# taindp98/Endoscopy-Image-Classification

Measured on AMD Instinct MI355X. Metric: unlabeled images/sec/node (FixMatch ViT-S, 224², μ=7), higher is better.
Workload: dtype bf16; 1 GPU; F1: FixMatch ViT-S/16 step, global B=64 labeled + mu*B=448 unlabeled weak/strong pairs (64 + 448 per GPU, strong scaling), 224^2, C=23, tau=0.95, lambda_u=1, Adam 1e-3, EMA 0.999; global_batch=960, seq_len=197, parallelism=dp1, hipgraph=False

## Files before the change

### endoscopy-image-classification_amd/csrc/gemm.hip

```cpp
#include <algorithm>
#include <mutex>
#include <type_traits>

#include <hip/hip_ext.h>

#include "common.h"

namespace es_gemm {

constexpr int BM = 128, BN = 128, BK = 64;

enum Epi {
  EPI_BF16 = 0,
  EPI_GELU = 1,
  EPI_F32_RESID = 2,
  EPI_DGELU = 3,
  EPI_F32 = 4,
  EPI_PATCH = 5,
  EPI_GELU_ACT = 6,
  EPI_GELU_D = 7,
  EPI_MULAUX = 8,
};

struct NTArgs {
// ... 1405 lines not shown
        }
        if constexpr (s == 0)
          if (q == RPS / 2 - 1) load_resid(std::integral_constant<int, 3>{});
        const LnRow384 o = ln_row384(v, (q & 1) == 0, l.eps, gam_lds, bet_lds, lane);
        const int m = m0 + tile_row(s, q);
        const bool ok = m < p.M;
#pragma unroll
        for (int j = 0; j < 3; ++j) {
          const int c = (j * 64 + lane) * 2;
          __builtin_amdgcn_raw_buffer_store_b64(__builtin_bit_cast(u32x2, v[j]), rx,
                                                ok ? (unsigned)(m * p.ldc + c) * 4u : ES_OOB, 0, 0);
          __builtin_amdgcn_raw_buffer_store_b32(o.h[j], rh, ok ? (unsigned)(m * l.ldh + c) * 2u : ES_OOB, 0, 0);
        }
        const bool one = ok && lane == 0;
        __builtin_amdgcn_raw_buffer_store_b32(__builtin_bit_cast(unsigned, o.mean), rm,
                                              one ? (unsigned)m * 4u : ES_OOB, 0, 0);
        __builtin_amdgcn_raw_buffer_store_b32(__builtin_bit_cast(unsigned, o.rstd), rs,
                                              one ? (unsigned)m * 4u : ES_OOB, 0, 0);
      }
    };
    slab(std::integral_constant<int, 0>{});
    asm volatile("s_waitcnt lgkmcnt(0)" ::: "memory");
    __builtin_amdgcn_s_barrier();
    slab(std::integral_constant<int, 1>{});
    if (tid == 0) qslot[0] = claimed;
    asm volatile("s_waitcnt lgkmcnt(0)" ::: "memory");
    __builtin_amdgcn_s_barrier();
    cur = __builtin_amdgcn_readfirstlane(qslot[0]);
  }
  TILE_CTR_RELEASE(ctr, tid)
}
#undef TILE_CTR_RELEASE

#define NT_LAUNCH(E, BKT_, NST_, TBM_, ...)                                             \
  {                                                                                        \
    const size_t lds = std::max((size_t)NST_ * (TBM_ + BN) * BKT_ * 2, (size_t)4 * EPI_WAVE_BYTES); \
    allow_lds(gemm_nt_kernel<E, BKT_, NST_, TBM_, ##__VA_ARGS__>, lds);                   \
    hipLaunchKernelGGL(HIP_KERNEL_NAME(gemm_nt_kernel<E, BKT_, NST_, TBM_, ##__VA_ARGS__>), dim3(grid), dim3(256), lds, stream, a); \
    return ES_OK;                                                                          \
  }
#define NT_EPIS(BKT_, NST_, TBM_, ...)                                            \
  switch (epi) {                                                                  \
    case EPI_BF16: NT_LAUNCH(EPI_BF16, BKT_, NST_, TBM_, ##__VA_ARGS__)           \
    case EPI_GELU: NT_LAUNCH(EPI_GELU, BKT_, NST_, TBM_, ##__VA_ARGS__)           \
    case EPI_F32_RESID: NT_LAUNCH(EPI_F32_RESID, BKT_, NST_, TBM_, ##__VA_ARGS__) \
    case EPI_DGELU: NT_LAUNCH(EPI_DGELU, BKT_, NST_, TBM_, ##__VA_ARGS__)         \
    case EPI_F32: NT_LAUNCH(EPI_F32, BKT_, NST_, TBM_, ##__VA_ARGS__)             \
    case EPI_PATCH: NT_LAUNCH(EPI_PATCH, BKT_, NST_, TBM_, ##__VA_ARGS__)         \
    case EPI_GELU_ACT: NT_LAUNCH(EPI_GELU_ACT, BKT_, NST_, TBM_, ##__VA_ARGS__)   \
    case EPI_GELU_D: NT_LAUNCH(EPI_GELU_D, BKT_, NST_, TBM_, ##__VA_ARGS__)       \
    case EPI_MULAUX: NT_LAUNCH(EPI_MULAUX, BKT_, NST_, TBM_, ##__VA_ARGS__)       \
    default: return ES_BAD_ARG;                                                   \
  }
int launch_nt(int cfg, int epi, int grid, hipStream_t stream, const NTArgs& a) {
  if (cfg == 11 && epi == EPI_F32_RESID) NT_LAUNCH(EPI_F32_RESID, 64, 2, 64, 0)
  switch (cfg) {
    case 0: NT_EPIS(64, 2, 128)
    case 5: NT_EPIS(32, 2, 128)
    case 11: NT_EPIS(64, 2, 64)
    default: NT_EPIS(32, 3, 128)
  }
}
#undef NT_EPIS
#undef NT_LAUNCH

#define BIG_LAUNCH(E, WM_, MF_, NF_, NST_, BKT_, OCC_, ...)                                        \
// ... 39 lines not shown
  if (n < CTR_SLOTS) {
    tab[n] = s;
    return n++;
  }
  return (int)(((uintptr_t)s >> 6) % CTR_SLOTS);
}
static int persistent_grid(int tiles) {
  static const int cus = [] {
    int dev = 0, n = 0;
    (void)hipGetDevice(&dev);
    return (hipDeviceGetAttribute(&n, hipDeviceAttributeMultiprocessorCount, dev) != hipSuccess || n <= 0) ? 256 : n;
  }();
  return std::max(1, std::min(cus, tiles));
}

int launch_resid_ln(hipStream_t stream, const NTArgs& a, const RLArgs& l) {
  const int grid = persistent_grid((a.M + rlg::R - 1) / rlg::R);
  allow_lds(gemm_resid_ln_kernel, (size_t)rlg::LDS);
  hipLaunchKernelGGL(gemm_resid_ln_kernel, dim3(grid), dim3(512), rlg::LDS, stream, a, l, tile_ctr_slot(stream));
  return hipGetLastError() == hipSuccess ? ES_OK : ES_HIP_ERROR;
}

int launch_nt_ln(int ring, hipStream_t stream, const NTArgs& a, const RLArgs& l) {
  const int grid = persistent_grid((a.M + nlg::TBM - 1) / nlg::TBM);
  const int slot = tile_ctr_slot(stream);
  constexpr size_t lds3 = nlg::lds<3, 32>(), lds2 = nlg::lds<2, 64>();
  if (ring == 1) {
    allow_lds(gemm_nt_ln_kernel<3, 32>, lds3);
    hipLaunchKernelGGL(HIP_KERNEL_NAME(gemm_nt_ln_kernel<3, 32>), dim3(grid), dim3(512), lds3, stream, a, l, slot);
  } else {
    allow_lds(gemm_nt_ln_kernel<2, 64>, lds2);
    hipLaunchKernelGGL(HIP_KERNEL_NAME(gemm_nt_ln_kernel<2, 64>), dim3(grid), dim3(512), lds2, stream, a, l, slot);
  }
  return hipGetLastError() == hipSuccess ? ES_OK : ES_HIP_ERROR;
}

}
using namespace es_gemm;

static int g_gemm_variant = -1;
static int g_tn_variant = -1;
static int g_small_tile = 1;

extern "C" {

int es_gemm_tn_ex(const void* A1, int ld1, const void* A2, int ld2, int M, int N1, int N2, int splits,
                  float* workspace, float* out, int accumulate, float* bias_out, int variant, hipStream_t stream);

int es_gemm_nt(int epi, const void* A, int lda, const void* B, int ldb, const float* bias, void* C,
               int ldc, void* C2, const void* aux, int ldaux, int M, int N, int K, int np,
               hipStream_t stream) {
  if (M <= 0 || N <= 0 || K <= 0 || (N % BN) || (K % BK) || (lda % 8) || (ldb % 8) || (ldc % 4))
    return ES_BAD_SHAPE;
  if (!A || !B || !C) return ES_BAD_ARG;
  if (((epi == EPI_GELU || epi == EPI_GELU_D) && !C2) ||
      ((epi == EPI_F32_RESID || epi == EPI_DGELU || epi == EPI_MULAUX || epi == EPI_PATCH) && !aux))
    return ES_BAD_ARG;
  if (epi == EPI_PATCH && np <= 0) return ES_BAD_ARG;
  if ((epi == EPI_F32_RESID || epi == EPI_PATCH) && ((ldaux % 4) || ldaux < N)) return ES_BAD_SHAPE;
  if ((epi == EPI_DGELU || epi == EPI_MULAUX) && ((ldaux % 8) || ldaux < N)) return ES_BAD_SHAPE;
  NTArgs a{(const bf16*)A, (const bf16*)B, bias, C, C2, aux, M, N, K, lda, ldb, ldc, ldaux, np};
  int variant = g_gemm_variant;
  if (variant < 0) {
    const bool gelu = epi == EPI_GELU || epi == EPI_GELU_ACT || epi == EPI_GELU_D;
    const bool plain = epi == EPI_BF16 || epi == EPI_F32 || epi == EPI_F32_RESID || epi == EPI_MULAUX;
    if (g_small_tile && N <= 384 && ((K <= 384 && epi == EPI_F32_RESID) || (M < 32768 && (plain || epi == EPI_GELU_ACT))))
// ... 56 lines not shown
      (size_t)M * (size_t)std::max(ldc, ldaux) * 4 >= (1u << 31))
    return ES_BAD_SHAPE;
  if (!A || !B || !C || !aux || !gamma || !beta || !h || !mean || !rstd) return ES_BAD_ARG;
  if ((((uintptr_t)A | (uintptr_t)aux | (uintptr_t)B | (uintptr_t)gamma | (uintptr_t)beta) & 15) ||
      (bias && ((uintptr_t)bias & 15)) || ((uintptr_t)C & 7) || ((uintptr_t)h & 3))
    return ES_BAD_ARG;
  NTArgs a{(const bf16*)A, (const bf16*)B, bias, C, nullptr, aux, M, N, K, lda, ldb, ldc, ldaux, 0};
  RLArgs l{gamma, beta, (bf16*)h, mean, rstd, ldh, eps};
  return launch_resid_ln(stream, a, l);
}

static int g_nt_ln_ring = 0;
int es_gemm_nt_ln(const void* A, int lda, const void* B, int ldb, const float* bias, float* C, int ldc,
                  const float* aux, int ldaux, const float* gamma, const float* beta, void* h, int ldh, float* mean,
                  float* rstd, int M, int N, int K, float eps, hipStream_t stream) {
  if (M <= 0 || N != nlg::D || K <= 0 || (K % 64) || (lda % 8) || (ldb % 8) || (ldc % 2) || (ldaux % 2) || (ldh % 2) ||
      lda < K || ldb < K || ldc < N || ldaux < N || ldh < N ||
      (size_t)M * (size_t)std::max(std::max(ldc, ldaux), ldh) * 4 >= (1u << 31))
    return ES_BAD_SHAPE;
  if (!A || !B || !C || !aux || !gamma || !beta || !h || !mean || !rstd) return ES_BAD_ARG;
  if ((((uintptr_t)A | (uintptr_t)B | (uintptr_t)gamma | (uintptr_t)beta) & 15) || (bias && ((uintptr_t)bias & 15)) ||
      (((uintptr_t)C | (uintptr_t)aux) & 7) || (((uintptr_t)h | (uintptr_t)mean | (uintptr_t)rstd) & 3))
    return ES_BAD_ARG;
  NTArgs a{(const bf16*)A, (const bf16*)B, bias, C, nullptr, aux, M, N, K, lda, ldb, ldc, ldaux, 0};
  RLArgs l{gamma, beta, (bf16*)h, mean, rstd, ldh, eps};
  return launch_nt_ln(g_nt_ln_ring, stream, a, l);
}
int endossl_nt_ln_ring(int v) {
  const int old = g_nt_ln_ring;
  g_nt_ln_ring = v == 1 ? 1 : 0;
  return old;
}

static bool gemm_variant_ok(int v) {
  return v == -1 || v == 0 || v == 1 || v == 2 || v == 5 || v == 6 || v == 10 || v == 11;
}
int es_set_gemm_variant(int v) {
  if (!gemm_variant_ok(v)) return ES_BAD_ARG;
  const int old = g_gemm_variant;
  g_gemm_variant = v;
  return old;
}

int es_set_gemm_small_tile(int v) {
  const int old = g_small_tile;
  g_small_tile = v;
  return old;
}

int es_set_tn_variant(int v) {
  if (v != -1 && v != 0 && v != 7) return ES_BAD_ARG;
  const int old = g_tn_variant;
  g_tn_variant = v;
  return old;
}

constexpr int TN_MIN_SPLIT_TOKENS = 512;
static bool tn_big_ok(int N1, int N2, int ld1, int ld2) {
  return N1 % TB1 == 0 && N2 % TB2 == 0 && ld1 % 8 == 0 && ld2 % 8 == 0;
}
static int tn_pick(int M, int N1, int N2, int ld1, int ld2, int v) {
  if (!(N1 % BM == 0 && N2 % BN == 0)) return 7;
  if (v == 7) return tn_big_ok(N1, N2, ld1, ld2) ? 7 : 0;
  if (v >= 0) return 0;
  return (tn_big_ok(N1, N2, ld1, ld2) && M >= 65536) ? 7 : 0;
}
// ... 259 lines not shown
```

### endoscopy-image-classification_amd/endossl/_lib.py

```python
import ctypes
import os

import torch

_HERE = os.path.dirname(os.path.abspath(__file__))
LIB_PATH = os.environ.get("ENDOSSL_LIB", os.path.join(_HERE, "lib", "libendossl_hip.so"))

V, I, L, F, Z = ctypes.c_void_p, ctypes.c_int, ctypes.c_long, ctypes.c_float, ctypes.c_size_t
U64 = ctypes.c_ulonglong

SIGNATURES = {
    "es_abi_version": (I, []),
    "es_gemm_nt": (I, [I, V, I, V, I, V, V, I, V, V, I, I, I, I, I, V]),
    "es_gemm_nt_resid_ln": (I, [V, I, V, I, V, V, I, V, I, V, V, V, I, V, V, I, I, I, F, V]),
    "es_gemm_nt_ln": (I, [V, I, V, I, V, V, I, V, I, V, V, V, I, V, V, I, I, I, F, V]),
    "es_set_gemm_variant": (I, [I]),
    "es_set_gemm_small_tile": (I, [I]),
    "es_gemm_tn_workspace": (Z, [I, I, I]),
    "es_gemm_tn": (I, [V, I, V, I, I, I, I, I, V, V, I, V, V]),
    "es_gemm_tn_ex": (I, [V, I, V, I, I, I, I, I, V, V, I, V, I, V]),
    "es_set_tn_variant": (I, [I]),
    "es_set_attn_variant": (I, [I]),
    "es_set_attn_bwd_variant": (I, [I]),
    "es_set_attn_bwd_grid": (I, [I]),
    "es_set_ln_fwd_grid": (I, [I]),
    "es_set_attn_bwd_long": (I, [I]),
    "es_splitk_reduce": (I, [V, V, I, I, I, V]),
    "es_tn_problem_size": (Z, []),
    "es_gemm_tn_grouped_prepare": (I, [V, I]),
    "es_gemm_tn_grouped": (I, [V, I, I, V]),
    "es_set_stem_kernels": (I, [I]),
    "es_gemm_tn_big_grouped_table_bytes": (Z, [I]),
    "es_gemm_tn_big_grouped_workspace": (Z, [V, I, I]),
    "es_gemm_tn_big_grouped_prepare": (I, [V, I, I, V, Z, V, V]),
    "es_gemm_tn_big_grouped": (I, [V, I, V, V]),
    "es_gemm_tn_big_grouped_timed": (I, [V, I, V, V, V, V]),
    "es_event_create": (I, [V]),
    "es_event_elapsed": (I, [V, V, V]),
    "es_event_destroy": (I, [V]),
    "es_colsum": (I, [V, I, I, I, V, I, V, I, V]),
    "es_attn_fwd": (I, [V, I, V, I, V, I, I, I, F, V]),
    "es_attn_bwd": (I, [V, I, V, I, V, V, V, I, V, I, I, I, I, F, V]),
    "es_attn_cls_fwd": (I, [V, I, V, I, V, I, I, I, F, V]),
    "es_attn_cls_bwd": (I, [V, I, V, I, V, V, I, V, I, I, I, I, F, V]),
    "es_reduce_partials": (I, [V, V, I, I, I, V]),
    "es_layernorm_fwd": (I, [V, I, V, V, V, I, V, V, I, I, F, V]),
    "es_layernorm_bwd": (I, [V, I, V, I, V, V, V, V, I, V, I, V, I, V, V, V, I, I, I, I, V]),
    "es_layernorm_bwd_b16": (I, [V, I, V, I, V, V, V, V, I, V, I, V, I, V, V, V, I, I, I, I, V]),
# ... 250 lines not shown
```

### endoscopy-image-classification_amd/endossl/block.py

```python
import contextlib
import ctypes

import torch

from . import _lib
from ._lib import ptr, stream

EPI_BF16, EPI_GELU, EPI_F32_RESID, EPI_DGELU, EPI_F32, EPI_PATCH, EPI_GELU_ACT, EPI_GELU_D, EPI_MULAUX = range(9)
ATTN_SCALE = 64 ** -0.5


def gemm_nt(call, epi, a, w, bias, c, M, N, K, c2=None, aux=None, ldc=None, ldaux=None, npatch=0, s=None):
    call("es_gemm_nt", epi, ptr(a), a.stride(0), ptr(w), w.stride(0), ptr(bias), ptr(c), ldc or c.stride(0), ptr(c2),
         ptr(aux), 0 if aux is None else ldaux or aux.stride(0), M, N, K, npatch, stream() if s is None else s)


def gemm_nt_resid_ln(call, a, w, bias, xmid, xin, gamma, beta, h, mean, rstd, M, N, K, eps, s=None):
    call("es_gemm_nt_resid_ln", ptr(a), a.stride(0), ptr(w), w.stride(0), ptr(bias), ptr(xmid), xmid.stride(0),
         ptr(xin), xin.stride(0), ptr(gamma), ptr(beta), ptr(h), h.stride(0), ptr(mean), ptr(rstd), M, N, K, eps,
         stream() if s is None else s)


def gemm_nt_ln(call, a, w, bias, xout, xmid, gamma, beta, h, mean, rstd, M, N, K, eps, s=None):
    call("es_gemm_nt_ln", ptr(a), a.stride(0), ptr(w), w.stride(0), ptr(bias), ptr(xout), xout.stride(0), ptr(xmid),
         xmid.stride(0), ptr(gamma), ptr(beta), ptr(h), h.stride(0), ptr(mean), ptr(rstd), M, N, K, eps,
         stream() if s is None else s)


def layernorm_fwd(call, x, gamma, beta, y, mean, rstd, M, D, eps, s=None):
    call("es_layernorm_fwd", ptr(x), x.stride(0), ptr(gamma), ptr(beta), ptr(y), y.stride(0), ptr(mean), ptr(rstd), M,
         D, eps, stream() if s is None else s)


def layernorm_bwd(call, dy, x, mean, rstd, gamma, dres, dx, dxb, dgamma, dbeta, ws, blocks, M, D, accumulate,
                  lddx=None, s=None):
    call("es_layernorm_bwd_b16" if dy.dtype == torch.bfloat16 else "es_layernorm_bwd", ptr(dy), dy.stride(0), ptr(x),
         x.stride(0), ptr(mean), ptr(rstd), ptr(gamma), ptr(dres), dres.stride(0), ptr(dx), lddx or dx.stride(0),
         ptr(dxb), 0 if dxb is None else dxb.stride(0), ptr(dgamma), ptr(dbeta), ptr(ws), blocks, M, D, accumulate,
         stream() if s is None else s)


def attn_fwd(call, qkv, o, lse, n, T, H, s=None, cls=False):
    call("es_attn_cls_fwd" if cls else "es_attn_fwd", ptr(qkv), qkv.stride(0), ptr(o), o.stride(0), ptr(lse), n, T, H,
         ATTN_SCALE, stream() if s is None else s)


def attn_bwd(call, qkv, o, lse, delta, do, dqkv, n, T, H, s=None):
    call("es_attn_bwd", ptr(qkv), qkv.stride(0), ptr(o), o.stride(0), ptr(lse), ptr(delta), ptr(do), do.stride(0),
         ptr(dqkv), dqkv.stride(0), n, T, H, ATTN_SCALE, stream() if s is None else s)


def attn_cls_bwd(call, qkv, o, lse, do, dqkv, n, T, H, s=None):
    call("es_attn_cls_bwd", ptr(qkv), qkv.stride(0), ptr(o), o.stride(0), ptr(lse), ptr(do), do.stride(0), ptr(dqkv),
         dqkv.stride(0), n, T, H, ATTN_SCALE, stream() if s is None else s)


def cast_f32_bf16(call, src, dst, numel, s=None):
    call("es_cast_f32_bf16", ptr(src), ptr(dst), numel, stream() if s is None else s)

# ... 24 lines not shown
        w, bias = self.wb[b + "attn.qkv.weight"], p(b + "attn.qkv.bias")
        if cls is not None and split_q:
            gemm_nt(call, EPI_BF16, R.h1, w[D:], bias[D:], R.qkv[:, D:], M, 2 * D, D, s=s)
            cls.h1[:R.n].copy_(R.h1[:M].view(R.n, R.T, D)[:, 0])
            gemm_nt(call, EPI_BF16, cls.h1, w[:D], bias[:D], R.qkv, R.n, D, D, ldc=R.T * 3 * D, s=s)
        else:
            gemm_nt(call, EPI_BF16, R.h1, w, bias, R.qkv, M, 3 * D, D, s=s)
        Ro = R if cls is None else cls
        attn_fwd(call, R.qkv, Ro.o, Ro.lse, R.n, R.T, self.heads, s, cls is not None)

    def mlp_fwd(self, b, R, train, fused=False, label=None, next_ln=None):
        call, p, wb, s, M = self.call, self.p, self.wb, stream(), R.rows
        D, Hd = R.h2.shape[1], R.act.shape[1]
        if fused:
            gemm_nt_resid_ln(call, R.o, wb[b + "attn.proj.weight"], p(b + "attn.proj.bias"), R.xmid, R.x,
                             p(b + "norm2.weight"), p(b + "norm2.bias"), R.h2, R.mean2, R.rstd2, M, D, D, self.eps, s)
        else:
            gemm_nt(call, EPI_F32_RESID, R.o, wb[b + "attn.proj.weight"], p(b + "attn.proj.bias"), R.xmid, M, D, D,
                    aux=R.x, ldaux=R.ldx, s=s)
            layernorm_fwd(call, R.xmid, p(b + "norm2.weight"), p(b + "norm2.bias"), R.h2, R.mean2, R.rstd2, M, D,
                          self.eps, s)
        epi, c, c2 = (EPI_GELU_D if self.gelu_d else EPI_GELU, R.pre, R.act) if train else (EPI_GELU_ACT, R.act, None)
        fc1 = lambda: gemm_nt(call, epi, R.h2, wb[b + "mlp.fc1.weight"], p(b + "mlp.fc1.bias"), c, M, Hd, D,
                              c2=c2, s=s)
        self.bracket(label, 2.0 * M * Hd * D, fc1)
        if next_ln is not None:
            gamma, beta, h1, mean1, rstd1 = next_ln
            gemm_nt_ln(call, R.act, wb[b + "mlp.fc2.weight"], p(b + "mlp.fc2.bias"), R.out, R.xmid, gamma, beta, h1,
                       mean1, rstd1, M, D, Hd, self.eps, s)
            return
        gemm_nt(call, EPI_F32_RESID, R.act, wb[b + "mlp.fc2.weight"], p(b + "mlp.fc2.bias"), R.out, M, D, Hd,
                aux=R.xmid, s=s)

    def mlp_bwd(self, b, R, ln_bwd, wgrad=None, cap=nop, label=None):
        call, p, g, wt, s, M = self.call, self.p, self.g, self.wt, stream(), R.rows
        D, Hd = R.dxb.shape[1], R.dpre.shape[1]
        cap("b_dxb", R.dxb)
        gemm_nt(call, EPI_MULAUX if self.gelu_d else EPI_DGELU, R.dxb, wt[b + "mlp.fc2.weight"], None, R.dpre, M, Hd, D,
                aux=R.pre, s=s)
        if wgrad is not None:
            wgrad(R.dxb, D, R.act, Hd, M, g(b + "mlp.fc2.weight"), g(b + "mlp.fc2.bias"))
        gemm_nt(call, self.epi_dh, R.dpre, wt[b + "mlp.fc1.weight"], None, R.dh, M, D, Hd, s=s)
        if wgrad is not None:
            wgrad(R.dpre, Hd, R.h2, D, M, g(b + "mlp.fc1.weight"), g(b + "mlp.fc1.bias"), label=label)
        cap("b_dpre", R.dpre)
        cap("b_dh2", R.dh)
        ln_bwd(R.dh, R.xmid, R.mean2, R.rstd2, p(b + "norm2.weight"), R.dres, R.dxm, R.dxmb, g(b + "norm2.weight"),
               g(b + "norm2.bias"), M, lddx=R.lddxm)
        gemm_nt(call, EPI_BF16, R.dxmb, wt[b + "attn.proj.weight"], None, R.do, M, D, D, s=s)
        if wgrad is not None:
            wgrad(R.dxmb, D, R.o, D, M, g(b + "attn.proj.weight"), g(b + "attn.proj.bias"))
        cap("b_dxm", R.dxm, R.dxmb)
        cap("b_do", R.do)

    def attn_bwd(self, b, R, ln_bwd, wgrad=None, before_ln1=nop, cap=nop, cls=None, split_q=False):
        call, p, g, s, M, T = self.call, self.p, self.g, stream(), R.rows, R.T
        D = R.dh1.shape[1]
        if cls is None:
            attn_bwd(call, R.qkv, R.o, R.lse, R.delta, R.do, R.dqkv, R.n, T, self.heads, s)
        else:
            attn_cls_bwd(call, R.qkv, cls.o, cls.lse, cls.do, R.dqkv, R.n, T, self.heads, s)
        gemm_nt(call, self.epi_dh, R.dqkv, self.wt[b + "attn.qkv.weight"], None, R.dh1, M, D, 3 * D, s=s)
        if wgrad is not None:
            gw, gb = g(b + "attn.qkv.weight"), g(b + "attn.qkv.bias")
            if cls is not None and split_q:
                wgrad(R.dqkv[:, D:], 2 * D, R.h1, D, M, gw[D * D:], gb[D:], ld1=3 * D)
                wgrad(R.dqkv, D, R.h1, D, R.n, gw[:D * D], gb[:D], ld1=T * 3 * D, ld2=T * D)
            else:
                wgrad(R.dqkv, 3 * D, R.h1, D, M, gw, gb)
        cap("b_dqkv", R.dqkv)
        cap("b_dh1", R.dh1)
        before_ln1()
        ln_bwd(R.dh1, R.x, R.mean1, R.rstd1, p(b + "norm1.weight"), R.dxm, R.dx, R.dxb_next, g(b + "norm1.weight"),
               g(b + "norm1.bias"), M)

# ... 42 lines not shown
```

### endoscopy-image-classification_amd/endossl/vit.py

```python
import ctypes
import functools
import math
import os

import torch
import torch.nn as nn

from . import _lib, block
from ._lib import call, ptr
from .block import (EPI_BF16, EPI_DGELU, EPI_F32, EPI_F32_RESID, EPI_GELU, EPI_GELU_ACT,
                    EPI_GELU_D, EPI_MULAUX, EPI_PATCH, Rows, _TNProblem)

LN_BWD_BLOCKS = 1024
SIDE_PRIORITY = -1
SIDE_PRIORITY_MIN_M = 65536


IMAGENET_MEAN = (0.485, 0.456, 0.406)
IMAGENET_STD = (0.229, 0.224, 0.225)


def _rup(x, m):
    return (x + m - 1) // m * m

# ... 213 lines not shown
            self._launch_grouped(self.problems, 0)
        if self.defer:
            self._ln_flush(self.defer)
        if self.side is not None:
            self.main.wait_stream(self.side)


class Engine:

    TN_TARGET_BLOCKS = 768
    TN_SHARE = 0.5
    TN_SHARE_MIN_M = 16384
    TN_MAX_SPLITS = 128
    GROUP_WGRAD = "auto"
    GROUP_WGRAD_MAX_M = 16384
    GROUP_LAYERS = 6
    DEFER_LN_GRADS = True
    LN_MULTI_MAX = 32
    LAYER_WGRAD = True
    LAYER_TN_SHARE = 0.375
    _OV = os.environ.get("ENDOSSL_OVERLAP", "1")
    OVERLAP_FWD = _OV in ("1", "fwd")
    OVERLAP = _OV in ("1", "bwd")
    DH_BF16 = True
    GELU_D = True
    PRUNE_LAST = True
    PRUNE_Q = True
    RESID_LN = os.environ.get("ENDOSSL_RESID_LN", "1") == "1"
    RESID_LN_MIN_M = 40000
    FC2_LN = os.environ.get("ENDOSSL_FC2_LN", "1") == "1"
    FC2_LN_MIN_M = 50000
    FC2_LN_TRAIN = True
    FC2_LN_WEAK = True

    PARITY_NAMES = {n: n + "_f32" for n in (
        "es_gemm_nt", "es_gemm_tn", "es_attn_fwd", "es_attn_bwd", "es_attn_cls_fwd", "es_attn_cls_bwd",
        "es_layernorm_fwd", "es_layernorm_bwd", "es_patch_im2col", "es_patch_im2col_u8", "es_embed_bwd",
        "es_pack_weights")}
    PARITY_NAMES.update({"es_layernorm_bwd_b16": "es_layernorm_bwd_f32", "es_cast_f32_bf16": "es_copy_f32"})

    def __init__(self, cfg, device, precision="bf16"):
        if precision not in ("bf16", "fp32"):
            raise ValueError(f"precision must be 'bf16' (production) or 'fp32' (parity mode), got {precision!r}")
        self.cfg, self.device = cfg, device
        self.precision = precision
        self.op_dtype = torch.bfloat16 if precision == "bf16" else torch.float32
        self.layout, self.offs, self.numel = param_layout(cfg)
        self.shapes = dict(self.layout)
        self._acts = {}
        self._grads = {}
        self._ws = None
        self._ws_ln = None
        self._ws_lnp = None
        self._lnp_next = 0
        self._side = None
        self._ncu_cache = None
        self._gtab = {}
        self._grad_b = None
        self.overlap = self.OVERLAP
        self.overlap_fwd = self.OVERLAP_FWD
        self._packed_version = -1
        D, Hd = cfg.dim, cfg.hidden
        b16 = self.op_dtype
        mats = [("patch_embed.proj.weight", D, 3 * cfg.patch * cfg.patch, False)]
        for i in range(cfg.depth):
            b = f"blocks.{i}."
# ... 201 lines not shown
        if defer is not None and grid >= 64:
            ws = self.ln_part_workspace(self._lnp_next)
            self._lnp_next += 1
            block.layernorm_bwd(self._call, dy, x, mean, rstd, gamma, dres, dx, dxb, None, None, ws, LN_BWD_BLOCKS, M,
                                D, 0, lddx)
            defer.append((ws, dgamma, dbeta, grid, 0))
            return
        block.layernorm_bwd(self._call, dy, x, mean, rstd, gamma, dres, dx, dxb, dgamma, dbeta, self.ln_workspace(),
                            LN_BWD_BLOCKS, M, D, 0, lddx)

    def ln_part_workspace(self, k):
        if self._ws_lnp is None:
            self._ws_lnp = []
        while len(self._ws_lnp) <= k:
            self._ws_lnp.append(torch.empty(2 * LN_BWD_BLOCKS * self.cfg.dim, dtype=torch.float32, device=self.device))
        return self._ws_lnp[k]

    def _ln_grads_flush(self, pending):
        if not pending:
            return
        lib = _lib.load()
        esz = lib.es_ln_param_grads_entry_size()
        for c0 in range(0, len(pending), self.LN_MULTI_MAX):
            chunk = pending[c0:c0 + self.LN_MULTI_MAX]
            raw = (ctypes.c_char * (esz * len(chunk)))()
            for j, (ws, dg, db, grid, acc) in enumerate(chunk):
                ent = (ctypes.c_void_p(ptr(ws)), ctypes.c_void_p(ptr(dg)), ctypes.c_void_p(ptr(db)),
                       ctypes.c_int(grid), ctypes.c_int(self.cfg.dim), ctypes.c_int(acc), ctypes.c_int(0))
                buf = b"".join(bytes(e) for e in ent)
                ctypes.memmove(ctypes.byref(raw, j * esz), buf, len(buf))
            self._call("es_ln_param_grads_multi", ctypes.addressof(raw), len(chunk), _lib.stream())
        pending.clear()

    def backward(self, flat, grad, dlogits=None, dfts=None, zero_grad=True, grad_ready=None):
        cfg = self.cfg
        s = _lib.stream()
        top = dfts if cfg.head == "emb" else dlogits
        if top is None:
            raise ValueError("Engine.backward needs dlogits (cls head) or dfts (emb head)")
        n = int(top.shape[0])
        A = self.acts(n, True)
        D, T, M = cfg.dim, cfg.T, A.M
        gv = lambda name: self.view(grad, name)
        fv = lambda name: self.view(flat, name)
        grouped = self._grouped_wgrad(M, grad_ready)
        GS = self._grad_sets(n, grouped)
        G = GS[0]
        sched = _WgradSchedule(
            GS, M, cfg.depth, grouped, layer_wgrad=self.LAYER_WGRAD, defer_ln=self.DEFER_LN_GRADS,
            bf16=self.precision == "bf16", capture=self.capture is not None, group_layers=self.GROUP_LAYERS,
            min_m=self.TN_SHARE_MIN_M, main=torch.cuda.current_stream(self.device),
            side=self.side_stream(M) if self.overlap else None, wgrad=self._wgrad, wgrad_layer=self._wgrad_layer,
            launch_grouped=self._launch_grouped, ln_flush=self._ln_grads_flush, grad_ready=grad_ready,
            block_range=self._block_range)
        self._lnp_next = 0
        ln_bwd = functools.partial(self._ln_bwd, defer=sched.defer)
        if zero_grad and cfg.head == "emb":
            grad.zero_()
        prune = self._prune()
        GL = sched.grad_sets(cfg.depth - 1)[0]
        dtop, Tt = (GL.c_dx, 1) if prune else (G.dx, T)
        if not prune:
            G.dx.zero_()
        if cfg.head == "emb":
            dfts = dfts.contiguous()
            self._call("es_cls_ln_bwd", ptr(dfts), D, ptr(fv("norm.weight")), ptr(A.xhat), ptr(A.rstd_cls), ptr(dtop), D, Tt,
                 ptr(gv("norm.weight")), ptr(gv("norm.bias")), n, D, s)
        else:
            dlogits = dlogits.contiguous()
            self._call("es_cls_head_bwd_ex", ptr(dlogits), cfg.num_classes, ptr(fv("head.weight")), ptr(fv("norm.weight")),
                 ptr(fv("norm.bias")), ptr(A.xhat), ptr(A.rstd_cls), ptr(G.dyn), ptr(dtop), D, Tt,
                 ptr(gv("head.weight")), ptr(gv("head.bias")), ptr(gv("norm.weight")), ptr(gv("norm.bias")), n, D,
                 cfg.num_classes, 0 if zero_grad else 1, s)
        if self.capture is not None:
            self.capture("dtop", True, cfg.depth - 1, dtop[:n] if prune else G.dx[:M])
        if prune:
            block.cast_f32_bf16(self._call, GL.c_dx, GL.c_dxb, n * D)
        else:
            block.cast_f32_bf16(self._call, G.dx, GL.dxb, M * D)
        ch = self._chain(flat, grad)
        cap = block.nop
        for i in reversed(range(cfg.depth)):
            b = f"blocks.{i}."
            Gi, Gn = sched.grad_sets(i)
            before_ln1 = functools.partial(sched.before_ln1, i)
            if self.capture is not None:
                cap = functools.partial(self._capture_rows, i, M)
            R = self._bwd_rows(A, G, Gi, Gn, i, n)
            if prune and i == cfg.depth - 1:
                Rc, R.dxm = self._cls_rows(A, n, G=Gi), Gi.dxm_cls
                ch.mlp_bwd(b, Rc, ln_bwd, sched.wgrad)
                split_q = self.PRUNE_Q and self._split_q_rows(n, _lib.tn_variant())
                ch.attn_bwd(b, R, ln_bwd, sched.wgrad, before_ln1, cls=Rc, split_q=split_q)
            else:
                ch.mlp_bwd(b, R, ln_bwd, sched.wgrad, cap, label="fc1_wgrad")
                ch.attn_bwd(b, R, ln_bwd, sched.wgrad, before_ln1, cap)
            if self.capture is not None:
                self.capture("bwd", True, i, G.dx[:M])
            sched.block_done(i)
        self._call("es_embed_bwd", ptr(G.dx), D, ptr(G.dpatch), D, ptr(gv("pos_embed")), ptr(gv("cls_token")), n, T, D, 0,
             s)
        sched.wgrad(G.dpatch, D, A.patches, 3 * cfg.patch * cfg.patch, n * cfg.np, gv("patch_embed.proj.weight"),
                    gv("patch_embed.proj.bias"))
        sched.finish()
        return grad

    def _grad_sets(self, n, grouped):
        mk = lambda: _Grads(self.cfg, n, self.device, self.op_dtype)
        if n not in self._grads:
            self._grads[n] = (mk(), mk())
        if not grouped:
            return self._grads[n]
        key = (n, "grouped")
        if key not in self._grads:
            self._grads[key] = [self._grads[n][0]] + [mk() for _ in range(self.cfg.depth)]
        return self._grads[key]

    def _block_range(self, i):
        nxt = f"blocks.{i + 1}.norm1.weight" if i + 1 < self.cfg.depth else "norm.weight"
        return self.offs[f"blocks.{i}.norm1.weight"], self.offs[nxt]

    def _capture_rows(self, i, M, kind, *ts):
        self.capture(kind, True, i, *(t[:M] for t in ts))

    def _bwd_rows(self, A, G, Gi, Gn, i, n):
        return Rows(n, self.cfg.T, self.cfg.heads, dxb=Gi.dxb, pre=A.pre[i], act=A.act[i], dpre=Gi.dpre, dh=G.dh,
                    h2=A.h2[i], xmid=A.xmid[i], mean2=A.mean2[i], rstd2=A.rstd2[i], dres=G.dx, dxm=G.dxm, dxmb=Gi.dxmb,
                    do=G.do, o=A.o[i], qkv=A.qkv[i], lse=A.lse[i], delta=G.delta, dqkv=Gi.dqkv, dh1=G.dh, h1=A.h1[i],
# ... 166 lines not shown
```

### include/endossl.h

```cpp
#ifndef ENDOSSL_H
#define ENDOSSL_H
#include <stddef.h>
#include <stdint.h>
#include <hip/hip_runtime_api.h>

#ifdef __cplusplus
extern "C" {
#endif

int es_abi_version(void);

int es_gemm_nt(int epi, const void* A, int lda, const void* B, int ldb, const float* bias, void* C, int ldc,
               void* C2, const void* aux, int ldaux, int M, int N, int K, int np, hipStream_t stream);
int es_gemm_nt_resid_ln(const void* A, int lda, const void* B, int ldb, const float* bias, float* C, int ldc,
                        const float* aux, int ldaux, const float* gamma, const float* beta, void* h, int ldh,
                        float* mean, float* rstd, int M, int N, int K, float eps, hipStream_t stream);
int es_gemm_nt_ln(const void* A, int lda, const void* B, int ldb, const float* bias, float* C, int ldc,
                  const float* aux, int ldaux, const float* gamma, const float* beta, void* h, int ldh, float* mean,
                  float* rstd, int M, int N, int K, float eps, hipStream_t stream);
int es_set_gemm_variant(int variant);
int es_set_gemm_small_tile(int v);
int es_set_tn_variant(int variant);
size_t es_gemm_tn_workspace(int N1, int N2, int splits);
int es_gemm_tn(const void* A1, int ld1, const void* A2, int ld2, int M, int N1, int N2, int splits,
               float* workspace, float* out, int accumulate, float* bias_out, hipStream_t stream);
int es_gemm_tn_ex(const void* A1, int ld1, const void* A2, int ld2, int M, int N1, int N2, int splits,
                  float* workspace, float* out, int accumulate, float* bias_out, int variant, hipStream_t stream);
int es_splitk_reduce(const float* P, float* out, int S, int n, int accumulate, hipStream_t stream);
typedef struct {
  const void* dy;
  const void* x;
  float* out;
  float* bias_out;
  int M, N1, N2, ld1, ld2;
  int mchunk, tile0, pad;
} es_tn_problem;
size_t es_tn_problem_size(void);
int es_gemm_tn_grouped_prepare(void* host_table, int count);
int es_gemm_tn_grouped(const void* device_table, int count, int total_tiles, hipStream_t stream);
size_t es_gemm_tn_big_grouped_table_bytes(int count);
size_t es_gemm_tn_big_grouped_workspace(const void* problems, int count, int target_wgs);
int es_gemm_tn_big_grouped_prepare(const void* problems, int count, int target_wgs, float* workspace,
                                   size_t workspace_floats, void* table, int* dims);
int es_gemm_tn_big_grouped(const void* table, int count, const int* dims, hipStream_t stream);
int es_gemm_tn_big_grouped_timed(const void* table, int count, const int* dims, void* start, void* stop,
                                 hipStream_t stream);
int es_event_create(void** ev);
int es_event_elapsed(void* start, void* stop, float* ms);
int es_event_destroy(void* ev);
int es_colsum(const void* Y, int ld, int M, int N, float* workspace, int blocks, float* out, int accumulate,
              hipStream_t stream);
int es_reduce_partials(const float* P, float* out, int G, int N, int accumulate, hipStream_t stream);
// ... 393 lines not shown
```

Baseline: 15300 unlabeled images/s.

## Fuse MLP backward fc2 dgrad and fc1 dgrad into one chunked kernel

Adds a kernel that, for each 128-row tile, computes dpre = (dx·W2ᵀ)⊙GELU' in 64-column hidden chunks kept in LDS, and immediately accumulates dh = dpre·W1ᵀ. The weights stream through a four-slot ring while dpre is still written out for the fc1 weight-gradient. This drops the second GEMM's read of dpre from HBM and one kernel launch per block. The cost is a non-persistent, one-block-per-CU kernel holding large accumulators, which could lower occupancy. It is enabled by default for large M with dim 384 and hidden 1536.

```diff
diff --git a/endoscopy-image-classification_amd/csrc/gemm.hip b/endoscopy-image-classification_amd/csrc/gemm.hip
--- a/endoscopy-image-classification_amd/csrc/gemm.hip
+++ b/endoscopy-image-classification_amd/csrc/gemm.hip
@@ -1461,6 +1461,201 @@
 }
 #undef TILE_CTR_RELEASE
 
+namespace mdg {
+constexpr int TBM = 128, D = 384, HD = 1536, HC = 64;
+constexpr int PANEL = TBM * 128;
+constexpr int XA = (D / 64) * PANEL, CH = PANEL;
+constexpr int AUXB = TBM * HC * 2;
+constexpr int UNIT = 8192, NSLOT = 4;
+constexpr int LDS = XA + CH + AUXB + NSLOT * UNIT;
+constexpr int U1 = D / 64, NS = D / 128, U2 = (HC / 32) * NS, UPC = U1 + U2, NCH = HD / HC;
+constexpr int UPS = 1, SPC = UPC / UPS, LA = NSLOT / UPS - 1, S1 = U1 / UPS;
+constexpr int WW = 4;
+constexpr int WPU = UNIT / 1024 / WW;
+constexpr int XPC = AUXB / 1024 / (8 - WW);
+static_assert(UPC % NSLOT == 0 && NSLOT % UPS == 0 && U1 % UPS == 0 && LA >= 1 && S1 >= 1 && LDS <= 160 * 1024 &&
+              HC == 64 && WPU * WW * 1024 == UNIT && XPC * (8 - WW) * 1024 == AUXB, "ring / tile");
+}
+
+struct MDArgs {
+  const bf16* A; const bf16* W2; const bf16* W1; const bf16* aux;
+  bf16* dpre; bf16* dh;
+  int M, lda, ldw2, ldw1, ldaux, ldpre, lddh;
+};
+
+template <int STAUX>
+__global__ __launch_bounds__(512, 1) void gemm_nt_mlp_dgrad_kernel(MDArgs p) {
+  using namespace mdg;
+  extern __shared__ __attribute__((aligned(16))) char smem[];
+  char* const xa = smem;
+  char* const ch = smem + XA;
+  char* const auxb = ch + CH;
+  char* const ring = auxb + AUXB;
+  const int tid = threadIdx.x, lane = tid & 63;
+  const int w = __builtin_amdgcn_readfirstlane(tid >> 6);
+  const int wm1 = w >> 1, wn1 = w & 1;
+  const int wm = w >> 2, wn = w & 3;
+  const int g = lane >> 4, r = lane & 15;
+  const int m0 = blockIdx.x * TBM, last = p.M - 1;
+
+  const __amdgpu_buffer_rsrc_t rpre = buf_rsrc(p.dpre, (unsigned)p.M * p.ldpre * 2u);
+  const bool xwave = w >= WW;
+  const bf16* gx[XPC];
+#pragma unroll
+  for (int j = 0; j < XPC; ++j) {
+    const int row = ((w - WW) * XPC + j) * 8 + (lane >> 3);
+    gx[j] = p.aux + (size_t)min(m0 + row, last) * p.ldaux + swz128(row, lane & 7) * 8;
+  }
+  auto issue_aux = [&](int c) {
+#pragma unroll
+    for (int j = 0; j < XPC; ++j) glds16(gx[j] + c * HC, auxb + ((w - WW) * XPC + j) * 1024);
+  };
+  const bf16* g2[WPU];
+  const bf16* g1[WPU];
+#pragma unroll
+  for (int h = 0; h < WPU; ++h) {
+    const int blk = w + h * WW, r2 = blk * 8 + (lane >> 3), r1 = blk * 16 + (lane >> 2);
+    g2[h] = p.W2 + (size_t)r2 * p.ldw2 + swz128(r2, lane & 7) * 8;
+    g1[h] = p.W1 + (size_t)r1 * p.ldw1 + swz64(r1, lane & 3) * 8;
+  }
+  auto issue = [&](int c, int t) {
+    char* const dst = ring + (t % NSLOT) * UNIT + w * 1024;
+#pragma unroll
+    for (int h = 0; h < WPU; ++h) {
+      if (t < U1) {
+        glds16(g2[h] + (size_t)(c * HC) * p.ldw2 + t * 64, dst + h * WW * 1024);
+      } else {
+        const int ks = (t - U1) / NS, ns = (t - U1) % NS;
+        glds16(g1[h] + (size_t)(ns * 128) * p.ldw1 + c * HC + ks * 32, dst + h * WW * 1024);
+      }
+    }
+  };
+
+  f32x4 acc1[2][2], acc2[NS][4][2];
+#pragma unroll
+  for (int i = 0; i < 4; ++i)
+#pragma unroll
+    for (int j = 0; j < 2; ++j) {
+      if (i < 2) acc1[i][j] = f32x4{0.f, 0.f, 0.f, 0.f};
+#pragma unroll
+      for (int s = 0; s < NS; ++s) acc2[s][i][j] = f32x4{0.f, 0.f, 0.f, 0.f};
+    }
+
+#pragma unroll
+  for (int j = 0; j < XA / 1024 / 8; ++j) {
+    const int I = j * 8 + w, row = (I & 15) * 8 + (lane >> 3);
+    glds16(p.A + (size_t)min(m0 + row, last) * p.lda + (I >> 4) * 64 + swz128(row, lane & 7) * 8, xa + I * 1024);
+  }
+  asm volatile("" ::: "memory");
+  if (xwave) {
+    issue_aux(0);
+    wait_vmcnt_any(XPC);
+  } else {
+#pragma unroll
+    for (int t = 0; t < LA * UPS; ++t) issue(0, t);
+  }
+
+  bf16x8 af2[4];
+  for (int c = 0; c < NCH; ++c) {
+#pragma unroll
+    for (int st = 0; st < SPC; ++st) {
+      if (!xwave) wait_vmcnt_any((LA - 1) * UPS * WPU);
+      else if (st == S1 - 1) asm volatile("s_waitcnt vmcnt(0)" ::: "memory");
+      if (st == S1) asm volatile("s_waitcnt lgkmcnt(0)" ::: "memory");
+      __builtin_amdgcn_s_barrier();
+      if (!xwave) {
+#pragma unroll
+        for (int u = 0; u < UPS; ++u) {
+          const int t2 = (st + LA) * UPS + u;
+          const int tt = t2 < UPC ? t2 : t2 - UPC;
+          const int cc = t2 < UPC ? c : c + 1;
+          issue(min(cc, NCH - 1), tt);
+        }
+      }
+      if (st == S1 && xwave) {
+#pragma unroll
+        for (int j = 0; j < XPC; ++j) {
+          const int q = j * (8 - WW) * 64 + tid - WW * 64, row = q >> 3, pc = q & 7;
+          const u32x4 v = *(const u32x4*)(ch + row * 128 + swz128(row, pc) * 16);
+          const int m = m0 + row;
+          __builtin_amdgcn_raw_buffer_store_b128(
+              v, rpre, m < p.M ? (unsigned)(m * p.ldpre + c * HC + pc * 8) * 2u : ES_OOB, 0, STAUX);
+        }
+        issue_aux(min(c + 1, NCH - 1));
+      }
+#pragma unroll
+      for (int u = 0; u < UPS; ++u) {
+      const int t = st * UPS + u;
+      const char* const slot = ring + (t % NSLOT) * UNIT;
+      if (t < U1) {
+        const char* const As = xa + t * PANEL;
+#pragma unroll
+        for (int kk = 0; kk < 2; ++kk) {
+          bf16x8 af[2], bfr[2];
+#pragma unroll
+          for (int i = 0; i < 2; ++i) {
+            const int ra = wm1 * 32 + i * 16 + r, rb = wn1 * 32 + i * 16 + r;
+            af[i] = *(const bf16x8*)(As + ra * 128 + swz128(ra, kk * 4 + g) * 16);
+            bfr[i] = *(const bf16x8*)(slot + rb * 128 + swz128(rb, kk * 4 + g) * 16);
+          }
+#pragma unroll
+          for (int i = 0; i < 2; ++i)
+#pragma unroll
+            for (int j = 0; j < 2; ++j) acc1[i][j] = mfma16(bfr[j], af[i], acc1[i][j]);
+        }
+        if (t == U1 - 1) {
+#pragma unroll
+          for (int mi = 0; mi < 2; ++mi)
+#pragma unroll
+            for (int ni = 0; ni < 2; ++ni) {
+              const int row = wm1 * 32 + mi * 16 + r, col = wn1 * 32 + ni * 16 + 4 * g;
+              const int at = row * 128 + swz128(row, col >> 3) * 16 + (col & 7) * 2;
+              const bf16x4 gp = *(const bf16x4*)(auxb + at);
+              bf16x4 o;
+#pragma unroll
+              for (int i = 0; i < 4; ++i) o[i] = (bf16)((acc1[mi][ni][i] + 0.f) * (float)gp[i]);
+              *(bf16x4*)(ch + at) = o;
+              acc1[mi][ni] = f32x4{0.f, 0.f, 0.f, 0.f};
+            }
+        }
+      } else {
+        const int ks = (t - U1) / NS, ns = (t - U1) % NS;
+        bf16x8 bfr[2];
+#pragma unroll
+        for (int j = 0; j < 2; ++j) {
+          const int rb = wn * 32 + j * 16 + r;
+          bfr[j] = *(const bf16x8*)(slot + rb * 64 + swz64(rb, g) * 16);
+        }
+        if (ns == 0) {
+#pragma unroll
+          for (int i = 0; i < 4; ++i) {
+            const int ra = wm * 64 + i * 16 + r;
+            af2[i] = *(const bf16x8*)(ch + ra * 128 + swz128(ra, ks * 4 + g) * 16);
+          }
+        }
+#pragma unroll
+        for (int i = 0; i < 4; ++i)
+#pragma unroll
+          for (int j = 0; j < 2; ++j) acc2[ns][i][j] = mfma16(bfr[j], af2[i], acc2[ns][i][j]);
+      }
+      }
+    }
+  }
+
+  asm volatile("s_waitcnt vmcnt(0)" ::: "memory");
+  NTArgs q{};
+  q.C = p.dh;
+  q.M = p.M;
+  q.N = D;
+  q.ldc = p.lddh;
+#pragma unroll
+  for (int s = 0; s < NS; ++s) {
+    const int mw0 = m0 + wm * 64, nw0 = s * 128 + wn * 32;
+    const EpiPre<EPI_BF16, 2> e = epi_prefetch<EPI_BF16, 2>(q, mw0, nw0, lane);
+    staged_epilogue_g<EPI_BF16, 4, 2, STAUX>(q, xa + w * epi_wave_bytes<2>(), acc2[s], mw0, nw0, lane, e);
+  }
+}
+
 #define NT_LAUNCH(E, BKT_, NST_, TBM_, ...)                                             \
   {                                                                                        \
     const size_t lds = std::max((size_t)NST_ * (TBM_ + BN) * BKT_ * 2, (size_t)4 * EPI_WAVE_BYTES); \
@@ -1566,6 +1761,13 @@
     allow_lds(gemm_nt_ln_kernel<2, 64>, lds2);
     hipLaunchKernelGGL(HIP_KERNEL_NAME(gemm_nt_ln_kernel<2, 64>), dim3(grid), dim3(512), lds2, stream, a, l, slot);
   }
+  return hipGetLastError() == hipSuccess ? ES_OK : ES_HIP_ERROR;
+}
+
+int launch_mlp_dgrad(hipStream_t stream, const MDArgs& a) {
+  const int grid = (a.M + mdg::TBM - 1) / mdg::TBM;
+  allow_lds(gemm_nt_mlp_dgrad_kernel<2>, (size_t)mdg::LDS);
+  hipLaunchKernelGGL(HIP_KERNEL_NAME(gemm_nt_mlp_dgrad_kernel<2>), dim3(grid), dim3(512), mdg::LDS, stream, a);
   return hipGetLastError() == hipSuccess ? ES_OK : ES_HIP_ERROR;
 }
 
@@ -1688,6 +1890,21 @@
   return old;
 }
 
+int es_gemm_mlp_dgrad(const void* dxb, int lda, const void* w2t, int ldw2, const void* w1t, int ldw1, const void* aux,
+                      int ldaux, void* dpre, int ldpre, void* dh, int lddh, int M, int D, int Hd,
+                      hipStream_t stream) {
+  if (M <= 0 || D != mdg::D || Hd != mdg::HD || (lda % 8) || (ldw2 % 8) || (ldw1 % 8) || (ldaux % 8) || (ldpre % 8) ||
+      (lddh % 8) || lda < D || ldw2 < D || lddh < D || ldw1 < Hd || ldaux < Hd || ldpre < Hd ||
+      (size_t)M * (size_t)std::max(std::max(ldaux, ldpre), std::max(lda, lddh)) * 2 >= (1u << 31))
+    return ES_BAD_SHAPE;
+  if (!dxb || !w2t || !w1t || !aux || !dpre || !dh) return ES_BAD_ARG;
+  if (((uintptr_t)dxb | (uintptr_t)w2t | (uintptr_t)w1t | (uintptr_t)aux | (uintptr_t)dpre | (uintptr_t)dh) & 15)
+    return ES_BAD_ARG;
+  MDArgs a{(const bf16*)dxb, (const bf16*)w2t, (const bf16*)w1t, (const bf16*)aux, (bf16*)dpre, (bf16*)dh,
+           M, lda, ldw2, ldw1, ldaux, ldpre, lddh};
+  return launch_mlp_dgrad(stream, a);
+}
+
 static bool gemm_variant_ok(int v) {
   return v == -1 || v == 0 || v == 1 || v == 2 || v == 5 || v == 6 || v == 10 || v == 11;
 }
diff --git a/endoscopy-image-classification_amd/endossl/_lib.py b/endoscopy-image-classification_amd/endossl/_lib.py
--- a/endoscopy-image-classification_amd/endossl/_lib.py
+++ b/endoscopy-image-classification_amd/endossl/_lib.py
@@ -14,6 +14,7 @@
     "es_gemm_nt": (I, [I, V, I, V, I, V, V, I, V, V, I, I, I, I, I, V]),
     "es_gemm_nt_resid_ln": (I, [V, I, V, I, V, V, I, V, I, V, V, V, I, V, V, I, I, I, F, V]),
     "es_gemm_nt_ln": (I, [V, I, V, I, V, V, I, V, I, V, V, V, I, V, V, I, I, I, F, V]),
+    "es_gemm_mlp_dgrad": (I, [V, I, V, I, V, I, V, I, V, I, V, I, I, I, I, V]),
     "es_set_gemm_variant": (I, [I]),
     "es_set_gemm_small_tile": (I, [I]),
     "es_gemm_tn_workspace": (Z, [I, I, I]),
diff --git a/endoscopy-image-classification_amd/endossl/block.py b/endoscopy-image-classification_amd/endossl/block.py
--- a/endoscopy-image-classification_amd/endossl/block.py
+++ b/endoscopy-image-classification_amd/endossl/block.py
@@ -25,6 +25,11 @@
     call("es_gemm_nt_ln", ptr(a), a.stride(0), ptr(w), w.stride(0), ptr(bias), ptr(xout), xout.stride(0), ptr(xmid),
          xmid.stride(0), ptr(gamma), ptr(beta), ptr(h), h.stride(0), ptr(mean), ptr(rstd), M, N, K, eps,
          stream() if s is None else s)
+
+
+def gemm_mlp_dgrad(call, dxb, w2t, w1t, aux, dpre, dh, M, D, Hd, s=None):
+    call("es_gemm_mlp_dgrad", ptr(dxb), dxb.stride(0), ptr(w2t), w2t.stride(0), ptr(w1t), w1t.stride(0), ptr(aux),
+         aux.stride(0), ptr(dpre), dpre.stride(0), ptr(dh), dh.stride(0), M, D, Hd, stream() if s is None else s)
 
 
 def layernorm_fwd(call, x, gamma, beta, y, mean, rstd, M, D, eps, s=None):
@@ -115,15 +120,23 @@
         gemm_nt(call, EPI_F32_RESID, R.act, wb[b + "mlp.fc2.weight"], p(b + "mlp.fc2.bias"), R.out, M, D, Hd,
                 aux=R.xmid, s=s)
 
-    def mlp_bwd(self, b, R, ln_bwd, wgrad=None, cap=nop, label=None):
+    def mlp_bwd(self, b, R, ln_bwd, wgrad=None, cap=nop, label=None, fused_dgrad=False):
         call, p, g, wt, s, M = self.call, self.p, self.g, self.wt, stream(), R.rows
         D, Hd = R.dxb.shape[1], R.dpre.shape[1]
         cap("b_dxb", R.dxb)
-        gemm_nt(call, EPI_MULAUX if self.gelu_d else EPI_DGELU, R.dxb, wt[b + "mlp.fc2.weight"], None, R.dpre, M, Hd, D,
-                aux=R.pre, s=s)
-        if wgrad is not None:
-            wgrad(R.dxb, D, R.act, Hd, M, g(b + "mlp.fc2.weight"), g(b + "mlp.fc2.bias"))
-        gemm_nt(call, self.epi_dh, R.dpre, wt[b + "mlp.fc1.weight"], None, R.dh, M, D, Hd, s=s)
+        if fused_dgrad:
+            if not self.gelu_d or self.epi_dh != EPI_BF16:
+                raise ValueError("mlp_bwd(fused_dgrad=True) needs the GELU' form (gelu_d) and bf16 d(LN output)")
+            gemm_mlp_dgrad(call, R.dxb, wt[b + "mlp.fc2.weight"], wt[b + "mlp.fc1.weight"], R.pre, R.dpre, R.dh, M, D,
+                           Hd, s)
+            if wgrad is not None:
+                wgrad(R.dxb, D, R.act, Hd, M, g(b + "mlp.fc2.weight"), g(b + "mlp.fc2.bias"))
+        else:
+            gemm_nt(call, EPI_MULAUX if self.gelu_d else EPI_DGELU, R.dxb, wt[b + "mlp.fc2.weight"], None, R.dpre, M,
+                    Hd, D, aux=R.pre, s=s)
+            if wgrad is not None:
+                wgrad(R.dxb, D, R.act, Hd, M, g(b + "mlp.fc2.weight"), g(b + "mlp.fc2.bias"))
+            gemm_nt(call, self.epi_dh, R.dpre, wt[b + "mlp.fc1.weight"], None, R.dh, M, D, Hd, s=s)
         if wgrad is not None:
             wgrad(R.dpre, Hd, R.h2, D, M, g(b + "mlp.fc1.weight"), g(b + "mlp.fc1.bias"), label=label)
         cap("b_dpre", R.dpre)
diff --git a/endoscopy-image-classification_amd/endossl/vit.py b/endoscopy-image-classification_amd/endossl/vit.py
--- a/endoscopy-image-classification_amd/endossl/vit.py
+++ b/endoscopy-image-classification_amd/endossl/vit.py
@@ -269,6 +269,8 @@
     FC2_LN_MIN_M = 50000
     FC2_LN_TRAIN = True
     FC2_LN_WEAK = True
+    MLP_DGRAD = os.environ.get("ENDOSSL_MLP_DGRAD", "1") == "1"
+    MLP_DGRAD_MIN_M = 50000
 
     PARITY_NAMES = {n: n + "_f32" for n in (
         "es_gemm_nt", "es_gemm_tn", "es_attn_fwd", "es_attn_bwd", "es_attn_cls_fwd", "es_attn_cls_bwd",
@@ -536,6 +538,11 @@
             self._call("es_ln_param_grads_multi", ctypes.addressof(raw), len(chunk), _lib.stream())
         pending.clear()
 
+    def _mlp_dgrad(self, M):
+        return bool(self.MLP_DGRAD and self.cfg.dim == 384 and self.cfg.hidden == 1536 and self.precision == "bf16"
+                    and self.GELU_D and self.DH_BF16 and M >= self.MLP_DGRAD_MIN_M
+                    and M * self.cfg.hidden * 2 < 2 ** 31)
+
     def backward(self, flat, grad, dlogits=None, dfts=None, zero_grad=True, grad_ready=None):
         cfg = self.cfg
         s = _lib.stream()
@@ -583,6 +590,7 @@
         else:
             block.cast_f32_bf16(self._call, G.dx, GL.dxb, M * D)
         ch = self._chain(flat, grad)
+        mlp_dgrad = self._mlp_dgrad(M)
         cap = block.nop
         for i in reversed(range(cfg.depth)):
             b = f"blocks.{i}."
@@ -597,7 +605,7 @@
                 split_q = self.PRUNE_Q and self._split_q_rows(n, _lib.tn_variant())
                 ch.attn_bwd(b, R, ln_bwd, sched.wgrad, before_ln1, cls=Rc, split_q=split_q)
             else:
-                ch.mlp_bwd(b, R, ln_bwd, sched.wgrad, cap, label="fc1_wgrad")
+                ch.mlp_bwd(b, R, ln_bwd, sched.wgrad, cap, label="fc1_wgrad", fused_dgrad=mlp_dgrad)
                 ch.attn_bwd(b, R, ln_bwd, sched.wgrad, before_ln1, cap)
             if self.capture is not None:
                 self.capture("bwd", True, i, G.dx[:M])
diff --git a/include/endossl.h b/include/endossl.h
--- a/include/endossl.h
+++ b/include/endossl.h
@@ -18,6 +18,8 @@
 int es_gemm_nt_ln(const void* A, int lda, const void* B, int ldb, const float* bias, float* C, int ldc,
                   const float* aux, int ldaux, const float* gamma, const float* beta, void* h, int ldh, float* mean,
                   float* rstd, int M, int N, int K, float eps, hipStream_t stream);
+int es_gemm_mlp_dgrad(const void* dxb, int lda, const void* w2t, int ldw2, const void* w1t, int ldw1, const void* aux,
+                      int ldaux, void* dpre, int ldpre, void* dh, int lddh, int M, int D, int Hd, hipStream_t stream);
 int es_set_gemm_variant(int variant);
 int es_set_gemm_small_tile(int v);
 int es_set_tn_variant(int variant);
```

Result: no change. 15450 unlabeled images/s, median of 6 (+1.0%).
